# dschleef/schroedinger

Measured on AMD Instinct MI355X. Metric: Mpix/s IIWT+OBMC decode, 2160p s16, higher is better.
Workload: dtype s16

## Files before the change

### schroedinger_amd/csrc/frameops.hip

```cpp

#include "schro_hip_internal.h"
#include <type_traits>

namespace schro {
namespace {

constexpr int kThreads = 256;

__device__ __forceinline__ int
clampi (int x, int lo, int hi)
{
  return min (max (x, lo), hi);
}


constexpr int kCvtTW = 512, kCvtTH = 4;

template < typename T >
__device__ __forceinline__ uint8_t
offsetconvert (T s)
{
  if constexpr (sizeof (T) == 2) {
    int v = (int16_t) (s + 128);
    return (uint8_t) clampi (v, 0, 255);
  } else {
    int t = (int) ((unsigned) s + 128u);
    t = clampi (t, -32768, 32767);
    return (uint8_t) clampi (t, 0, 255);
  }
}

template < typename T >
__global__ __launch_bounds__ (kThreads)
void convert_kernel (const ConvertJob * __restrict__ jobs, int njobs)
{
  const int bid = xcd_tile_id (blockIdx.x, gridDim.x);
  const ConvertJob job = jobs[find_job (jobs, njobs, bid)];
  const int t = bid - job.tile_base;
  const int tx = t % job.tiles_x, ty = t / job.tiles_x;
  const int x = tx * kCvtTW + (threadIdx.x % 64) * 8;
  const int y = ty * kCvtTH + threadIdx.x / 64;
  if (y >= job.h || x >= job.w)
    return;
  const T *s = (const T *) ((const char *) job.src + (size_t) y * job.src_stride) + x;
  uint8_t *d = job.dst + (size_t) y * job.dst_stride + x;
  const bool vec = x + 8 <= job.w && (((uintptr_t) s & 15) == 0) && (((uintptr_t) d & 7) == 0);
  if (job.pred) {
    const uint8_t *p = job.pred + (size_t) y * job.pred_stride + x;
    for (int e = 0; e < 8 && x + e < job.w; e++)
      gstore < uint8_t > (d + e, combine_pred < T > (gload < T > (s + e), gload < uint8_t > (p + e)));
    return;
  }
  if (vec) {
    T v[8];
    if constexpr (sizeof (T) == 2) {
      *reinterpret_cast < u32x4 * >(v) = gload < u32x4 > (s);
    } else {
      reinterpret_cast < u32x4 * >(v)[0] = gload < u32x4 > (s);
      reinterpret_cast < u32x4 * >(v)[1] = gload < u32x4 > (s + 4);
    }
    uint32_t lo = 0, hi = 0;
#pragma unroll
    for (int e = 0; e < 4; e++) {
      lo |= (uint32_t) offsetconvert < T > (v[e]) << (8 * e);
      hi |= (uint32_t) offsetconvert < T > (v[4 + e]) << (8 * e);
    }
    gstore < u32x2 > (d, (u32x2) { lo, hi });
  } else {
    for (int e = 0; e < 8 && x + e < job.w; e++)
      gstore < uint8_t > (d + e, offsetconvert < T > (gload < T > (s + e)));
  }
}


constexpr int kUpTW = 128, kUpTH = 16;

typedef short short2v __attribute__ ((ext_vector_type (2)));

__device__ __forceinline__ short2v
lo_pair (uint32_t d)
{
  return __builtin_bit_cast (short2v, __builtin_amdgcn_perm (0u, d, 0x0c010c00u));
}

__device__ __forceinline__ short2v
hi_pair (uint32_t d)
{
  return __builtin_bit_cast (short2v, __builtin_amdgcn_perm (0u, d, 0x0c030c02u));
}

__device__ __forceinline__ short2v
mas8_pk (const short2v * r)
{
  short2v x = (r[3] + r[4]) * (short) 21 - (r[2] + r[5]) * (short) 7 + (r[1] + r[6]) * (short) 3
      - (r[0] + r[7]);
  x = (x + (short) 16) >> 5;
  x = __builtin_elementwise_max (x, (short2v) { 0, 0 });
  x = __builtin_elementwise_min (x, (short2v) { 255, 255 });
  return x;
}

__device__ __forceinline__ int
mas8_bytes (uint32_t lo4, uint32_t hi4)
{
  int acc = __builtin_amdgcn_sdot4 ((int) lo4, (int) 0x15f903ffu, 4096 + 16, false);
  acc = __builtin_amdgcn_sdot4 ((int) hi4, (int) 0xff03f915u, acc, false);
  return clampi (acc >> 5, 0, 255);
}

__device__ __forceinline__ void
mas8_row4 (uint32_t d0, uint32_t d1, uint32_t d2, int *out)
{
  out[0] = mas8_bytes (__builtin_amdgcn_alignbyte (d1, d0, 1), __builtin_amdgcn_alignbyte (d2, d1, 1));
  out[1] = mas8_bytes (__builtin_amdgcn_alignbyte (d1, d0, 2), __builtin_amdgcn_alignbyte (d2, d1, 2));
  out[2] = mas8_bytes (__builtin_amdgcn_alignbyte (d1, d0, 3), __builtin_amdgcn_alignbyte (d2, d1, 3));
  out[3] = mas8_bytes (d1, d2);
}

constexpr int kUpMaxLD = 2 * (kUpTW / 8 + 8);

template < bool PAIR > constexpr int kUpFetch = ((kUpTH + 7) * ((PAIR ? 2 : 1) * ((PAIR ? kUpTW / 2 : kUpTW) / 4 + 8) / 4) + kThreads - 1) / kThreads;

template < bool PAIR >
__device__ __forceinline__ void
upsample_fetch (const UpsampleJob & job, int t, u32x4 * q_out)
{
  constexpr int kTWp = PAIR ? kUpTW / 2 : kUpTW, kHalfLD = kTWp / 4 + 8;
  constexpr int kUpCh = (PAIR ? 2 : 1) * kHalfLD / 4, kHalfCh = kHalfLD / 4;
  const int tx = t % job.tiles_x, ty = t / job.tiles_x;
  const int x0 = tx * kTWp, y0 = ty * kUpTH;
  const int w = job.w, h = job.h;
  const int tid = threadIdx.x;
#pragma unroll
  for (int n = 0; n < kUpFetch < PAIR >; n++) {
    const int it = tid + n * kThreads;
    q_out[n] = (u32x4) { 0u, 0u, 0u, 0u };
    if (it >= (kUpTH + 7) * kUpCh)
      continue;
    const int ly = it / kUpCh, c = it - ly * kUpCh;
    const int half = PAIR ? c / kHalfCh : 0, cc = c - half * kHalfCh;
    const uint8_t *src = half ? job.src_b : job.src;
    const int sstride = half ? job.src_b_stride : job.src_stride;
    const bool src_al = ((((uintptr_t) src) | (uintptr_t) sstride) & 15) == 0;
    const int gy = clampi (y0 - 3 + ly, 0, h - 1);
    const int gx = x0 - 16 + 16 * cc;
    const uint8_t *row = src + (size_t) gy * sstride;
    u32x4 q;
    if (src_al && gx >= 0 && gx + 16 <= w) {
      q = gload < u32x4 > (row + gx);
    } else {
      uint32_t d[4] = { 0u, 0u, 0u, 0u };
#pragma unroll
      for (int k = 0; k < 16; k++)
        d[k >> 2] |= (uint32_t) gload < uint8_t > (row + clampi (gx + k, 0, w - 1)) << (8 * (k & 3));
      q = (u32x4) { d[0], d[1], d[2], d[3] };
    }
    q_out[n] = q;
  }
}

template < bool PAIR >
__device__ __forceinline__ void
upsample_stage (const u32x4 * q, uint32_t (*s0)[kUpMaxLD])
{
  constexpr int kTWp = PAIR ? kUpTW / 2 : kUpTW, kHalfLD = kTWp / 4 + 8, kUpCh = (PAIR ? 2 : 1) * kHalfLD / 4;
#pragma unroll
  for (int n = 0; n < kUpFetch < PAIR >; n++) {
    const int it = (int) threadIdx.x + n * kThreads;
    if (it < (kUpTH + 7) * kUpCh) {
      const int ly = it / kUpCh, c = it - ly * kUpCh;
      *reinterpret_cast < u32x4 * >(&s0[ly][4 * c]) = q[n];
    }
  }
}

template < bool PAIR >
__device__ __forceinline__ void
upsample_filter_store (const UpsampleJob & job, int t, uint32_t (*s0)[kUpMaxLD], uint32_t (*s2)[kUpMaxLD])
{
  constexpr int kTWp = PAIR ? kUpTW / 2 : kUpTW;
  constexpr int kHalfLD = kTWp / 4 + 8;
  constexpr int kHalfDW = kTWp / 4 + 2, kVDW = (PAIR ? 2 : 1) * kHalfDW;
  constexpr int ps = PAIR ? 1 : 0;
  static_assert ((PAIR ? 2 : 1) * kHalfLD <= kUpMaxLD, "LDS row");

  const int tx = t % job.tiles_x, ty = t / job.tiles_x;
  const int x0 = tx * kTWp, y0 = ty * kUpTH;
  const int w = job.w, h = job.h;
  const int tid = threadIdx.x;

  for (int it = tid; it < kUpTH * kVDW; it += kThreads) {
    const int gi = it % kVDW, ly = it / kVDW;
    const int half = PAIR ? gi / kHalfDW : 0, g = half * kHalfLD + (gi - half * kHalfDW) + 3;
    uint32_t out;
    if (y0 + ly >= h - 1) {
      out = s0[ly + 3][g];
    } else {
      short2v lo[8], hi[8];
#pragma unroll
      for (int k = 0; k < 8; k++) {
        const uint32_t d = s0[ly + k][g];
        lo[k] = lo_pair (d);
        hi[k] = hi_pair (d);
      }
      const short2v a = mas8_pk (lo), b = mas8_pk (hi);
      out = __builtin_amdgcn_perm (__builtin_bit_cast (uint32_t, b), __builtin_bit_cast (uint32_t, a), 0x06040200u);
    }
    s2[ly][g] = out;
  }
  __syncthreads ();

  static_assert ((kUpTW / 8) * kUpTH % kThreads == 0 && kUpTW / 8 == 16 && kUpTH % kHpBandRows == 0,
      "a lane per 8 pixels of 16 rows of the tile at a time");
  const int stride = job.dst_stride;
#pragma unroll 1
  for (int part = 0; part < (kUpTW / 8) * kUpTH / kThreads; part++) {
  const int ly = (tid >> 4) + part * (kThreads / 16), g8 = tid & 15;
  const int half = PAIR ? g8 >> 3 : 0, gg = PAIR ? g8 & 7 : g8;
  const int gx = x0 + 8 * gg, gy = y0 + ly;
  const int gd = half * kHalfLD + 2 * gg + 3;
  uint32_t pl[4][2];
  {
    const uint32_t a0 = s0[ly + 3][gd], a1 = s0[ly + 3][gd + 1], a2 = s0[ly + 3][gd + 2], a3 = s0[ly + 3][gd + 3];
    const uint32_t b0 = s2[ly][gd], b1 = s2[ly][gd + 1], b2 = s2[ly][gd + 2], b3 = s2[ly][gd + 3];
    constexpr uint32_t kS = 0x80808080u;
    int p1[8], p3[8];
    mas8_row4 (a0 ^ kS, a1 ^ kS, a2 ^ kS, p1);
    mas8_row4 (a1 ^ kS, a2 ^ kS, a3 ^ kS, p1 + 4);
    mas8_row4 (b0 ^ kS, b1 ^ kS, b2 ^ kS, p3);
    mas8_row4 (b1 ^ kS, b2 ^ kS, b3 ^ kS, p3 + 4);
    pl[0][0] = a1;
    pl[0][1] = a2;
    pl[2][0] = b1;
    pl[2][1] = b2;
    const bool edge_tile = x0 + kTWp >= w || y0 + kUpTH >= h;
#pragma unroll
    for (int hf = 0; hf < 2; hf++) {
      if (edge_tile) {
        pl[1][hf] = pl[3][hf] = 0;
#pragma unroll
        for (int e = 0; e < 4; e++) {
          const bool lastcol = gx + 4 * hf + e >= w - 1;
          int v1 = lastcol ? (int) ((pl[0][hf] >> (8 * e)) & 0xff) : p1[4 * hf + e];
          int v3 = lastcol ? (int) ((pl[2][hf] >> (8 * e)) & 0xff) : p3[4 * hf + e];
          if (gy >= h - 1)
            v3 = v1;
          pl[1][hf] |= (uint32_t) v1 << (8 * e);
          pl[3][hf] |= (uint32_t) v3 << (8 * e);
        }
      } else {
        pl[1][hf] = (uint32_t) p1[4 * hf] | ((uint32_t) p1[4 * hf + 1] << 8) | ((uint32_t) p1[4 * hf + 2] << 16)
            | ((uint32_t) p1[4 * hf + 3] << 24);
        pl[3][hf] = (uint32_t) p3[4 * hf] | ((uint32_t) p3[4 * hf + 1] << 8) | ((uint32_t) p3[4 * hf + 2] << 16)
            | ((uint32_t) p3[4 * hf + 3] << 24);
      }
    }
  }
  uint8_t *row = job.dst + hp_row_offset (min (gy, h - 1), stride);
  if constexpr (PAIR) {
    const int xb = 2 * (gx + kHpApron);
    const bool group_in = gx + 8 <= w;
#pragma unroll
    for (int p = 0; p < 4; p++) {
      const uint32_t n0 = (uint32_t) __builtin_amdgcn_mov_dpp ((int) pl[p][0], 0x128, 0xf, 0xf, true);
      const uint32_t n1 = (uint32_t) __builtin_amdgcn_mov_dpp ((int) pl[p][1], 0x128, 0xf, 0xf, true);
      if (group_in && gy < h) {
        const uint32_t u0 = half ? n0 : pl[p][0], u1 = half ? n1 : pl[p][1];
        const uint32_t v0 = half ? pl[p][0] : n0, v1 = half ? pl[p][1] : n1;
        const u32x4 v = (u32x4) { __builtin_amdgcn_perm (v0, u0, 0x05010400u), __builtin_amdgcn_perm (v0, u0, 0x07030602u),
          __builtin_amdgcn_perm (v1, u1, 0x05010400u), __builtin_amdgcn_perm (v1, u1, 0x07030602u) };
        gstore < u32x4 > (row + (size_t) ((xb >> 4) - half) * 512 + (size_t) (p * 128 + 16 * half), v);
      } else if (gy < h) {
        for (int e = 0; e < 8 && gx + e < w; e++) {
          const uint8_t v = (uint8_t) (pl[p][e >> 2] >> (8 * (e & 3)));
          const int xbe = xb + 2 * e + half;
          gstore < uint8_t > (row + hp_col_offset (xbe) + p * 128, v);
          gstore < uint8_t > (row + hp_col_offset (xbe - 16) + p * 128 + 16, v);
        }
      }
    }
  } else {
  const int odd = g8 & 1, xp16 = gx - 8 * odd + kHpApron;
  const bool pair_in = gx - 8 * odd + 16 <= w;
#pragma unroll
  for (int p = 0; p < 4; p++) {
    const uint32_t n0 = (uint32_t) __builtin_amdgcn_mov_dpp ((int) pl[p][0], 0xb1, 0xf, 0xf, true);
    const uint32_t n1 = (uint32_t) __builtin_amdgcn_mov_dpp ((int) pl[p][1], 0xb1, 0xf, 0xf, true);
    if (pair_in && gy < h) {
      const u32x4 v = odd ? (u32x4) { n0, n1, pl[p][0], pl[p][1] } : (u32x4) { pl[p][0], pl[p][1], n0, n1 };
      gstore < u32x4 > (row + (size_t) ((xp16 >> 4) - odd) * 512 + (size_t) (p * 128 + 16 * odd), v);
    } else if (gy < h) {
      for (int e = 0; e < 8 && gx + e < w; e++) {
        const uint8_t v = (uint8_t) (pl[p][e >> 2] >> (8 * (e & 3)));
        const int xp = gx + e + kHpApron;
        gstore < uint8_t > (row + hp_col_offset (xp) + p * 128, v);
        gstore < uint8_t > (row + hp_col_offset (xp - 16) + p * 128 + 16, v);
      }
    }
  }
  }
  }
  auto edge_dword = [&](int p, int r, int pos) {
    const uint32_t u = ((p < 2 ? s0[r + 3][pos >> 2] : s2[r][pos >> 2]) >> (8 * (pos & 3))) & 0xffu;
    if constexpr (!PAIR) {
      return u * 0x01010101u;
    } else {
      const uint32_t v = ((p < 2 ? s0[r + 3][kHalfLD + (pos >> 2)] : s2[r][kHalfLD + (pos >> 2)]) >> (8 * (pos & 3))) & 0xffu;
      return (u | (v << 8)) * 0x00010001u;
    }
  };
  if (x0 == 0) {
    constexpr int kPieces = 2 * ((kHpApron << ps) / 16) - 1;
    for (int it = tid; it < kUpTH * 4 * kPieces; it += kThreads) {
      const int piece = it % kPieces, p = (it / kPieces) & 3, r = it / (4 * kPieces);
      if (y0 + r >= h)
        continue;
      const uint32_t e = edge_dword (p, r, 16);
      uint8_t *d = job.dst + hp_row_offset (y0 + r, stride) + (size_t) ((piece >> 1) * 512 + 16 * (piece & 1)) + p * 128;
      gstore < u32x4 > (d, (u32x4) { e, e, e, e });
    }
  }
  if (x0 + kTWp >= w) {
    const int nch = stride >> 9, first = (w + kHpApron) << ps, c_lo = max (0, (first >> 4) - 1);
    const int ndw = (nch - c_lo) * 8;
    const int xl = w - 1 - (x0 - 16);
    for (int it = tid; it < kUpTH * 4 * ndw; it += kThreads) {
      const int dwi = it % ndw, p = (it / ndw) & 3, r = it / (4 * ndw);
      if (y0 + r >= h)
        continue;
      const int c = c_lo + (dwi >> 3), o = (dwi & 7) * 4, col = 16 * c + o;
      if (col + 3 < first)
        continue;
      const uint32_t e = edge_dword (p, r, xl);
      uint8_t *d = job.dst + hp_row_offset (y0 + r, stride) + (size_t) c * 512 + p * 128 + o;
      if (col >= first) {
        gstore < uint32_t > (d, e);
      } else {
        for (int k = first - col; k < 4; k++)
          gstore < uint8_t > (d + k, (uint8_t) (e >> (8 * k)));
      }
    }
  }
}

__global__ __launch_bounds__ (kThreads)
void upsample_kernel (const UpsampleJob * __restrict__ jobs, int njobs)
{
  __shared__ __attribute__ ((aligned (16))) uint32_t s0[kUpTH + 7][kUpMaxLD];
  __shared__ __attribute__ ((aligned (16))) uint32_t s2[kUpTH][kUpMaxLD];
  const int bid = xcd_tile_id (blockIdx.x, gridDim.x);
  const UpsampleJob job = jobs[find_job (jobs, njobs, bid)];
  if (job.src_b) {
    u32x4 q[kUpFetch < true >];
    upsample_fetch < true > (job, bid - job.tile_base, q);
    upsample_stage < true > (q, s0);
    __syncthreads ();
    upsample_filter_store < true > (job, bid - job.tile_base, s0, s2);
  } else {
    u32x4 q[kUpFetch < false >];
    upsample_fetch < false > (job, bid - job.tile_base, q);
    upsample_stage < false > (q, s0);
    __syncthreads ();
    upsample_filter_store < false > (job, bid - job.tile_base, s0, s2);
  }
}

#ifdef SCHRO_HIP_EXPERIMENTS
template < bool PAIR >
__device__ __forceinline__ void
upsample_persist_body (const UpsampleJob * __restrict__ jobs, int njobs, int total, uint32_t (*s0)[kUpMaxLD], uint32_t (*s2)[kUpMaxLD])
{
  u32x4 q[kUpFetch < PAIR >];
  int v = blockIdx.x;
  if (v >= total)
    return;
  int bid = xcd_tile_id (v, total);
  UpsampleJob job = jobs[find_job (jobs, njobs, bid)];
  upsample_fetch < PAIR > (job, bid - job.tile_base, q);
  for (;;) {
    upsample_stage < PAIR > (q, s0);
    __syncthreads ();
    const int vn = v + (int) gridDim.x;
    UpsampleJob jn = job;
    int bn = bid;
    if (vn < total) {
      bn = xcd_tile_id (vn, total);
      jn = jobs[find_job (jobs, njobs, bn)];
      upsample_fetch < PAIR > (jn, bn - jn.tile_base, q);
    }
    upsample_filter_store < PAIR > (job, bid - job.tile_base, s0, s2);
    if (vn >= total)
      break;
    __syncthreads ();
    v = vn;
    bid = bn;
    job = jn;
  }
}

__global__ __launch_bounds__ (kThreads)
void upsample_persist_kernel (const UpsampleJob * __restrict__ jobs, int njobs, int total)
{
  __shared__ __attribute__ ((aligned (16))) uint32_t s0[kUpTH + 7][kUpMaxLD];
  __shared__ __attribute__ ((aligned (16))) uint32_t s2[kUpTH][kUpMaxLD];
  if (jobs[0].src_b)
    upsample_persist_body < true > (jobs, njobs, total, s0, s2);
  else
    upsample_persist_body < false > (jobs, njobs, total, s0, s2);
}
#endif


constexpr int kPackGX = 64, kPackRows = 4;

__device__ __forceinline__ uint32_t
pack_sample (const PackJob & job, int comp, int t_hs, int X, int Y)
{
  int x, y;
  if (comp == 0) {
    x = min (X, job.sw - 1);
    y = min (Y, job.sh - 1);
  } else {
    const int sw = (job.sw + (1 << t_hs) - 1) >> t_hs;
    const int Xc = min (X, sw - 1), Yc = min (Y, job.sh - 1);
    x = t_hs == job.hs ? Xc : (t_hs > job.hs ? 2 * Xc : Xc >> 1);
    y = job.vs ? Yc >> 1 : Yc;
  }
  return gload < uint8_t > (job.src[comp] + (size_t) y * job.src_stride[comp] + x);
}

__device__ __forceinline__ uint32_t
v210_sample (const PackJob & job, int comp, int X, int Y)
{
  if (job.src_bpp == 1) {
    const uint32_t v = pack_sample (job, comp, 1, X, Y);
    return (v << 2) | (v >> 6);
  }
  const int cw = comp ? (job.sw + 1) >> 1 : job.sw;
  const int x = min (X, cw - 1), y = min (Y, job.sh - 1);
  const uint8_t *row = job.src[comp] + (size_t) y * job.src_stride[comp];
  const int v = job.src_bpp == 2 ? (int) gload < int16_t > ((const int16_t *) row + x)
      : (int) (int16_t) gload < int32_t > ((const int32_t *) row + x);
  return (uint32_t) clampi (v + 512, 0, 1023);
}

__device__ __forceinline__ int
wide_sample (const PackJob & job, int target_bpp, int t_hs, int comp, int X, int Y)
{
  const int cw = comp ? (job.sw + (1 << t_hs) - 1) >> t_hs : job.sw;
  const int x = min (X, cw - 1), y = min (Y, job.sh - 1);
  const uint8_t *row = job.src[comp] + (size_t) y * job.src_stride[comp];
  int v;
  if (job.src_bpp == 1)
    v = (int) gload < uint8_t > (row + x) - 128;
  else if (job.src_bpp == 2)
    v = gload < int16_t > ((const int16_t *) row + x);
  else
    v = gload < int32_t > ((const int32_t *) row + x);
  return target_bpp == 2 ? (int) (int16_t) v : v;
}

__device__ __forceinline__ uint32_t
v216_line_byte (const PackJob & job, int comp, int b, int Y)
{
  return ((uint32_t) (uint16_t) wide_sample (job, 2, 1, comp, b >> 1, Y) >> (8 * (b & 1))) & 0xffu;
}

__global__ __launch_bounds__ (kThreads)
void pack_kernel (const PackJob * __restrict__ jobs, int njobs)
{
  const int bid = xcd_tile_id (blockIdx.x, gridDim.x);
  const PackJob job = jobs[find_job (jobs, njobs, bid)];
  const int t = bid - job.tile_base;
  const int ty = fdiv (t, job.tiles_x), tx = t - ty * job.tiles_x;
  const int g = tx * kPackGX + (threadIdx.x & (kPackGX - 1));
  const int y = ty * kPackRows + (threadIdx.x >> 6);
  static_assert (kPackGX == 64 && kThreads == kPackGX * kPackRows, "one wave per packed row");
  if (y >= job.h)
    return;
  uint8_t *d = job.dst + (size_t) y * job.dst_stride + 16 * (size_t) g;
  uint32_t o[4];
  if (job.format == SCHRO_HIP_FORMAT_v210) {
    const int x0 = 6 * g;
    if (x0 >= job.w)
      return;
    uint32_t yv[6], cb[3], cr[3];
#pragma unroll
    for (int k = 0; k < 6; k++)
      yv[k] = x0 + k < job.w ? v210_sample (job, 0, x0 + k, y) : 0u;
#pragma unroll
    for (int k = 0; k < 3; k++) {
      const bool in = x0 + 2 * k < job.w;
      cb[k] = in ? v210_sample (job, 1, 3 * g + k, y) : 0u;
      cr[k] = in ? v210_sample (job, 2, 3 * g + k, y) : 0u;
    }
    o[0] = (cr[0] << 20) | (yv[0] << 10) | cb[0];
    o[1] = (yv[2] << 20) | (cb[1] << 10) | yv[1];
    o[2] = (cb[2] << 20) | (yv[3] << 10) | cr[1];
    o[3] = (yv[5] << 20) | (cr[2] << 10) | yv[4];
    if ((((uintptr_t) d) & 15) == 0) {
      gstore < u32x4 > (d, (u32x4) { o[0], o[1], o[2], o[3] });
    } else {
      for (int k = 0; k < 4; k++)
        gstore < u32_u > (d + 4 * k, o[k]);
    }
    return;
  }
  if (job.format == SCHRO_HIP_FORMAT_v216 || job.format == SCHRO_HIP_FORMAT_ARGB || job.format == SCHRO_HIP_FORMAT_AY64) {
    int nbytes = 16;
    if (job.format == SCHRO_HIP_FORMAT_v216) {
      const int pairs = job.w >> 1, j0 = 2 * g;
      if (j0 >= pairs)
        return;
#pragma unroll
      for (int k = 0; k < 2; k++) {
        const int j = j0 + k;
        const uint32_t u = v216_line_byte (job, 1, j, y), v = v216_line_byte (job, 2, j, y);
        const uint32_t y0 = v216_line_byte (job, 0, 2 * j, y), y1 = v216_line_byte (job, 0, 2 * j + 1, y);
        o[2 * k] = u * 0x0101u | (y0 * 0x0101u << 16);
        o[2 * k + 1] = v * 0x0101u | (y1 * 0x0101u << 16);
      }
      nbytes = 8 * min (2, pairs - j0);
    } else if (job.format == SCHRO_HIP_FORMAT_ARGB) {
      const int x0 = 4 * g;
      if (x0 >= job.w)
        return;
#pragma unroll
      for (int k = 0; k < 4; k++) {
        const int x = x0 + k;
        const int yv = wide_sample (job, 2, 0, 0, x, y), co = wide_sample (job, 2, 0, 1, x, y);
        const int cg = wide_sample (job, 2, 0, 2, x, y);
        const int t = yv + (cg >> 1), b = t - (co >> 1);
        o[k] = 0xffu | ((uint32_t) ((b + co) & 0xff) << 8) | ((uint32_t) ((t + cg) & 0xff) << 16)
            | ((uint32_t) (b & 0xff) << 24);
      }
      nbytes = 4 * min (4, job.w - x0);
    } else {
      const int x0 = 2 * g;
      if (x0 >= job.w)
        return;
#pragma unroll
      for (int k = 0; k < 2; k++) {
        const int x = x0 + k;
        uint32_t w[3];
#pragma unroll
        for (int c = 0; c < 3; c++) {
          const long long v = (long long) wide_sample (job, 4, 0, c, x, y) + 0x8000;
          w[c] = (uint32_t) (v < 0 ? 0 : (v > 0xffff ? 0xffff : v));
        }
        o[2 * k] = 0xffffu | (w[0] << 16);
        o[2 * k + 1] = w[1] | (w[2] << 16);
      }
      nbytes = 8 * min (2, job.w - x0);
    }
    if (nbytes == 16 && (((uintptr_t) d) & 15) == 0) {
      gstore < u32x4 > (d, (u32x4) { o[0], o[1], o[2], o[3] });
    } else {
      for (int b = 0; b < nbytes; b++)
        gstore < uint8_t > (d + b, (uint8_t) (o[b >> 2] >> (8 * (b & 3))));
    }
    return;
  }
  if (job.format == SCHRO_HIP_FORMAT_AYUV) {
    const int x0 = 4 * g;
    if (x0 >= job.w)
      return;
#pragma unroll
    for (int k = 0; k < 4; k++) {
      const int x = x0 + k;
      o[k] = 0xffu | (pack_sample (job, 0, 0, x, y) << 8) | (pack_sample (job, 1, 0, x, y) << 16)
          | (pack_sample (job, 2, 0, x, y) << 24);
    }
    const int n = min (4, job.w - x0);
    if (n == 4 && (((uintptr_t) d) & 15) == 0) {
      gstore < u32x4 > (d, (u32x4) { o[0], o[1], o[2], o[3] });
    } else {
      for (int k = 0; k < n; k++)
        for (int b = 0; b < 4; b++)
          gstore < uint8_t > (d + 4 * k + b, (uint8_t) (o[k] >> (8 * b)));
    }
  } else {
    const int p0 = 4 * g, pairs = job.w >> 1;
    if (p0 >= pairs)
      return;
    const bool yuyv = job.format == SCHRO_HIP_FORMAT_YUYV;
    const int cy = job.vs ? min (y, job.sh - 1) >> 1 : min (y, job.sh - 1);
    const uint8_t *py = job.src[0] + (size_t) min (y, job.sh - 1) * job.src_stride[0] + 2 * p0;
    const uint8_t *pu = job.src[1] + (size_t) cy * job.src_stride[1] + p0;
    const uint8_t *pv = job.src[2] + (size_t) cy * job.src_stride[2] + p0;
    if (job.hs == 1 && 2 * p0 + 8 <= job.sw && p0 + 4 <= pairs
        && ((((uintptr_t) py) & 7) | (((uintptr_t) pu) & 3) | (((uintptr_t) pv) & 3)) == 0) {
      const u32x2 yy = gload < u32x2 > (py);
      const uint32_t uu = gload < uint32_t > (pu), vv = gload < uint32_t > (pv);
      const uint32_t uv01 = __builtin_amdgcn_perm (vv, uu, 0x05010400u);
      const uint32_t uv23 = __builtin_amdgcn_perm (vv, uu, 0x07030602u);
      if (yuyv) {
        o[0] = __builtin_amdgcn_perm (uv01, yy.x, 0x05010400u);
        o[1] = __builtin_amdgcn_perm (uv01, yy.x, 0x07030602u);
        o[2] = __builtin_amdgcn_perm (uv23, yy.y, 0x05010400u);
        o[3] = __builtin_amdgcn_perm (uv23, yy.y, 0x07030602u);
      } else {
        o[0] = __builtin_amdgcn_perm (yy.x, uv01, 0x05010400u);
        o[1] = __builtin_amdgcn_perm (yy.x, uv01, 0x07030602u);
        o[2] = __builtin_amdgcn_perm (yy.y, uv23, 0x05010400u);
        o[3] = __builtin_amdgcn_perm (yy.y, uv23, 0x07030602u);
      }
      if ((((uintptr_t) d) & 15) == 0) {
        gstore < u32x4 > (d, (u32x4) { o[0], o[1], o[2], o[3] });
        return;
      }
    } else {
#pragma unroll
      for (int k = 0; k < 4; k++) {
        const int j = p0 + k;
        const uint32_t y0 = pack_sample (job, 0, 1, 2 * j, y), y1 = pack_sample (job, 0, 1, 2 * j + 1, y);
        const uint32_t u = pack_sample (job, 1, 1, j, y), v = pack_sample (job, 2, 1, j, y);
        o[k] = yuyv ? (y0 | (u << 8) | (y1 << 16) | (v << 24)) : (u | (y0 << 8) | (v << 16) | (y1 << 24));
      }
    }
    const int n = min (4, pairs - p0);
    for (int k = 0; k < n; k++)
      for (int b = 0; b < 4; b++)
        gstore < uint8_t > (d + 4 * k + b, (uint8_t) (o[k] >> (8 * b)));
  }
}

template < typename T >
__global__ __launch_bounds__ (kThreads)
void shift_right_kernel (const ConvertJob * __restrict__ jobs, int njobs, int shift)
{
  const int bid = blockIdx.x;
  const ConvertJob job = jobs[find_job (jobs, njobs, bid)];
  const int t = bid - job.tile_base;
  const int ty = fdiv (t, job.tiles_x), tx = t - ty * job.tiles_x;
  const int x = tx * kCvtTW + (threadIdx.x % 64) * 8;
  const int y = ty * kCvtTH + threadIdx.x / 64;
  if (y >= job.h || x >= job.w)
    return;
  typedef typename std::make_unsigned < T >::type U;
  const U rnd = (U) ((1u << shift) >> 1);
  T *row = (T *) ((char *) job.dst + (size_t) y * job.dst_stride);
  for (int e = 0; e < 8 && x + e < job.w; e++) {
    const T v = gload < T > (row + x + e);
    gstore < T > (row + x + e, (T) ((T) ((U) v + rnd) >> shift));
  }
}

template < typename S, bool SUB >
__global__ __launch_bounds__ (kThreads)
void add_kernel (const ConvertJob * __restrict__ jobs, int njobs)
{
  typedef short s16x2 __attribute__ ((ext_vector_type (2)));
  const int bid = blockIdx.x;
  const ConvertJob job = jobs[find_job (jobs, njobs, bid)];
  const int t = bid - job.tile_base;
  const int ty = fdiv (t, job.tiles_x), tx = t - ty * job.tiles_x;
  const int x = tx * kCvtTW + (threadIdx.x % 64) * 8;
  const int y = ty * kCvtTH + threadIdx.x / 64;
  if (y >= job.h || x >= job.w)
    return;
  int16_t *drow = (int16_t *) (job.dst + (size_t) y * job.dst_stride) + x;
  const S *srow = (const S *) ((const char *) job.src + (size_t) y * job.src_stride) + x;
  if (x + 8 <= job.w && (((uintptr_t) drow) & 15) == 0 && (((uintptr_t) srow) & (8 * sizeof (S) - 1)) == 0) {
    const u32x4 d = gload < u32x4 > (drow);
    uint32_t dv[4] = { d.x, d.y, d.z, d.w }, av[4];
    if constexpr (sizeof (S) == 2) {
      const u32x4 a = gload < u32x4 > (srow);
      av[0] = a.x;
      av[1] = a.y;
      av[2] = a.z;
      av[3] = a.w;
    } else {
      const u32x2 b = gload < u32x2 > (srow);
      av[0] = __builtin_amdgcn_perm (0u, b.x, 0x0c010c00u);
      av[1] = __builtin_amdgcn_perm (0u, b.x, 0x0c030c02u);
      av[2] = __builtin_amdgcn_perm (0u, b.y, 0x0c010c00u);
      av[3] = __builtin_amdgcn_perm (0u, b.y, 0x0c030c02u);
    }
#pragma unroll
    for (int k = 0; k < 4; k++) {
      const s16x2 a = __builtin_bit_cast (s16x2, dv[k]), b = __builtin_bit_cast (s16x2, av[k]);
      dv[k] = __builtin_bit_cast (uint32_t, (s16x2) (SUB ? a - b : a + b));
    }
    gstore < u32x4 > (drow, (u32x4) { dv[0], dv[1], dv[2], dv[3] });
    return;
  }
  for (int e = 0; e < 8 && x + e < job.w; e++) {
    const int16_t a = gload < int16_t > (drow + e), b = (int16_t) gload < S > (srow + e);
    gstore < int16_t > (drow + e, (int16_t) (SUB ? a - b : a + b));
  }
}

}

int
launch_shift_right (hipStream_t stream, const ConvertJob * d_jobs, int njobs, int total_tiles, int bpp, int shift)
{
  if (bpp == 2)
    SCHRO_LAUNCH ((shift_right_kernel < int16_t >), dim3 (total_tiles), dim3 (kThreads), 0, stream, d_jobs,
        njobs, shift);
  else
    SCHRO_LAUNCH ((shift_right_kernel < int32_t >), dim3 (total_tiles), dim3 (kThreads), 0, stream, d_jobs,
        njobs, shift);
  hipError_t e = hipGetLastError ();
  if (e != hipSuccess)
    return set_error (SCHRO_HIP_EDEVICE, "shift_right launch: %s", hipGetErrorString (e));
  return 0;
}

int
launch_add (hipStream_t stream, const ConvertJob * d_jobs, int njobs, int total_tiles, int src_bpp, bool subtract)
{
  if (src_bpp == 2 && subtract)
    SCHRO_LAUNCH ((add_kernel < int16_t, true >), dim3 (total_tiles), dim3 (kThreads), 0, stream, d_jobs, njobs);
  else if (subtract)
    SCHRO_LAUNCH ((add_kernel < uint8_t, true >), dim3 (total_tiles), dim3 (kThreads), 0, stream, d_jobs, njobs);
  else if (src_bpp == 2)
    SCHRO_LAUNCH ((add_kernel < int16_t, false >), dim3 (total_tiles), dim3 (kThreads), 0, stream, d_jobs, njobs);
  else
    SCHRO_LAUNCH ((add_kernel < uint8_t, false >), dim3 (total_tiles), dim3 (kThreads), 0, stream, d_jobs, njobs);
  hipError_t e = hipGetLastError ();
  if (e != hipSuccess)
    return set_error (SCHRO_HIP_EDEVICE, "add launch: %s", hipGetErrorString (e));
  return 0;
}

void
pack_tile_geometry (int *groups_x, int *rows)
{
  *groups_x = kPackGX;
  *rows = kPackRows;
}

int
launch_pack (hipStream_t stream, const PackJob * d_jobs, int njobs, int total_tiles)
{
  SCHRO_LAUNCH (pack_kernel, dim3 (total_tiles), dim3 (kThreads), 0, stream, d_jobs, njobs);
  hipError_t e = hipGetLastError ();
  if (e != hipSuccess)
    return set_error (SCHRO_HIP_EDEVICE, "pack launch: %s", hipGetErrorString (e));
  return 0;
}

void
convert_tile_geometry (int *tw, int *th)
{
  *tw = kCvtTW;
  *th = kCvtTH;
}

int
launch_convert (hipStream_t stream, const ConvertJob * d_jobs, int njobs, int total_tiles, int bpp)
{
  if (bpp == 2)
    SCHRO_LAUNCH ((convert_kernel < int16_t >), dim3 (total_tiles), dim3 (kThreads), 0,
        stream, d_jobs, njobs);
  else
    SCHRO_LAUNCH ((convert_kernel < int32_t >), dim3 (total_tiles), dim3 (kThreads), 0,
        stream, d_jobs, njobs);
  hipError_t e = hipGetLastError ();
  if (e != hipSuccess)
    return set_error (SCHRO_HIP_EDEVICE, "convert launch: %s", hipGetErrorString (e));
  return 0;
}

void
upsample_tile_geometry (int *tw, int *th)
{
  *tw = kUpTW;
  *th = kUpTH;
}

int
launch_upsample (hipStream_t stream, const UpsampleJob * d_jobs, int njobs, int total_tiles, int persist_grid)
{
#ifdef SCHRO_HIP_EXPERIMENTS
  if (persist_grid > 0 && persist_grid < total_tiles)
    SCHRO_LAUNCH (upsample_persist_kernel, dim3 (persist_grid), dim3 (kThreads), 0, stream, d_jobs, njobs, total_tiles);
  else
#endif
  SCHRO_LAUNCH (upsample_kernel, dim3 (total_tiles), dim3 (kThreads), 0, stream, d_jobs,
      njobs);
  hipError_t e = hipGetLastError ();
  if (e != hipSuccess)
    return set_error (SCHRO_HIP_EDEVICE, "upsample launch: %s", hipGetErrorString (e));
  return 0;
}

}
```

Baseline: 196,800.

## Restructure upsample filter: row-grouped vertical pass, early plane stores, packed clamps

The vertical half-pel pass now has each lane compute four output rows from eleven LDS reads, so loaded taps are reused across neighbouring rows instead of being reloaded eight times per row. The store phase drops its per-part loop and writes integer-position planes 0 and 2 before the horizontal filters run, so the global stores can overlap the arithmetic. Horizontal results are saturated with packed convert and v_sat_pk_u8_i16 instead of scalar clamps. Experiment-only env variants (stores-only and filters-only) and per-step template switches were added for profiling. One risk is that only part of the lanes are busy in the vertical pass.

```diff
diff --git a/schroedinger_amd/csrc/frameops.hip b/schroedinger_amd/csrc/frameops.hip
--- a/schroedinger_amd/csrc/frameops.hip
+++ b/schroedinger_amd/csrc/frameops.hip
@@ -1,5 +1,6 @@
 
 #include "schro_hip_internal.h"
+#include <cstring>
 #include <type_traits>
 
 namespace schro {
@@ -104,8 +105,7 @@
 mas8_bytes (uint32_t lo4, uint32_t hi4)
 {
   int acc = __builtin_amdgcn_sdot4 ((int) lo4, (int) 0x15f903ffu, 4096 + 16, false);
-  acc = __builtin_amdgcn_sdot4 ((int) hi4, (int) 0xff03f915u, acc, false);
-  return clampi (acc >> 5, 0, 255);
+  return __builtin_amdgcn_sdot4 ((int) hi4, (int) 0xff03f915u, acc, false);
 }
 
 __device__ __forceinline__ void
@@ -115,6 +115,28 @@
   out[1] = mas8_bytes (__builtin_amdgcn_alignbyte (d1, d0, 2), __builtin_amdgcn_alignbyte (d2, d1, 2));
   out[2] = mas8_bytes (__builtin_amdgcn_alignbyte (d1, d0, 3), __builtin_amdgcn_alignbyte (d2, d1, 3));
   out[3] = mas8_bytes (d1, d2);
+}
+
+__device__ __forceinline__ int
+mas8_sample (int sum)
+{
+  return clampi (sum >> 5, 0, 255);
+}
+
+__device__ __forceinline__ uint32_t
+sat_pair_u8 (short2v x)
+{
+  uint32_t r;
+  asm ("v_sat_pk_u8_i16 %0, %1":"=v" (r):"v" (__builtin_bit_cast (uint32_t, x)));
+  return r;
+}
+
+__device__ __forceinline__ uint32_t
+mas8_samples4 (const int *sum)
+{
+  const short2v lo = __builtin_amdgcn_cvt_pk_i16 (sum[0], sum[1]) >> (short2v) { 5, 5 };
+  const short2v hi = __builtin_amdgcn_cvt_pk_i16 (sum[2], sum[3]) >> (short2v) { 5, 5 };
+  return __builtin_amdgcn_perm (sat_pair_u8 (hi), sat_pair_u8 (lo), 0x05040100u);
 }
 
 constexpr int kUpMaxLD = 2 * (kUpTW / 8 + 8);
@@ -174,7 +196,12 @@
   }
 }
 
-template < bool PAIR >
+enum { kUpFull = 0, kUpStoresOnly = 1, kUpFiltersOnly = 2 };
+
+enum { kUpEarlyStores = 1, kUpRowGroups = 2, kUpPackedClamp = 4 };
+constexpr int kUpSteps = kUpEarlyStores | kUpRowGroups | kUpPackedClamp;
+
+template < bool PAIR, int MODE, int STEPS >
 __device__ __forceinline__ void
 upsample_filter_store (const UpsampleJob & job, int t, uint32_t (*s0)[kUpMaxLD], uint32_t (*s2)[kUpMaxLD])
 {
@@ -189,116 +216,147 @@
   const int w = job.w, h = job.h;
   const int tid = threadIdx.x;
 
-  for (int it = tid; it < kUpTH * kVDW; it += kThreads) {
-    const int gi = it % kVDW, ly = it / kVDW;
-    const int half = PAIR ? gi / kHalfDW : 0, g = half * kHalfLD + (gi - half * kHalfDW) + 3;
-    uint32_t out;
-    if (y0 + ly >= h - 1) {
-      out = s0[ly + 3][g];
-    } else {
-      short2v lo[8], hi[8];
-#pragma unroll
-      for (int k = 0; k < 8; k++) {
-        const uint32_t d = s0[ly + k][g];
-        lo[k] = lo_pair (d);
-        hi[k] = hi_pair (d);
-      }
-      const short2v a = mas8_pk (lo), b = mas8_pk (hi);
-      out = __builtin_amdgcn_perm (__builtin_bit_cast (uint32_t, b), __builtin_bit_cast (uint32_t, a), 0x06040200u);
-    }
-    s2[ly][g] = out;
+  static_assert ((kUpTW / 8) * kUpTH == kThreads && kUpTW / 8 == 16 && kUpTH % kHpBandRows == 0,
+      "a lane per 8 pixels of one row of the tile");
+  const int stride = job.dst_stride;
+  const int ly = tid >> 4, g8 = tid & 15;
+  const int shalf = PAIR ? g8 >> 3 : 0, gg = PAIR ? g8 & 7 : g8;
+  const int gx = x0 + 8 * gg, gy = y0 + ly;
+  const int gd = shalf * kHalfLD + 2 * gg + 3;
+  uint8_t *row = job.dst + hp_row_offset (min (gy, h - 1), stride);
+  uint32_t kept[4] = { 0u, 0u, 0u, 0u };
+  auto store_plane = [&](int p, uint32_t d0, uint32_t d1) {
+    if constexpr (MODE == kUpFiltersOnly) {
+      kept[p] = d0 ^ d1;
+    } else if constexpr (PAIR) {
+      const int xb = 2 * (gx + kHpApron);
+      const bool group_in = gx + 8 <= w;
+      const uint32_t n0 = (uint32_t) __builtin_amdgcn_mov_dpp ((int) d0, 0x128, 0xf, 0xf, true);
+      const uint32_t n1 = (uint32_t) __builtin_amdgcn_mov_dpp ((int) d1, 0x128, 0xf, 0xf, true);
+      if (group_in && gy < h) {
+        const uint32_t u0 = shalf ? n0 : d0, u1 = shalf ? n1 : d1;
+        const uint32_t v0 = shalf ? d0 : n0, v1 = shalf ? d1 : n1;
+        const u32x4 v = (u32x4) { __builtin_amdgcn_perm (v0, u0, 0x05010400u), __builtin_amdgcn_perm (v0, u0, 0x07030602u),
+          __builtin_amdgcn_perm (v1, u1, 0x05010400u), __builtin_amdgcn_perm (v1, u1, 0x07030602u) };
+        gstore < u32x4 > (row + (size_t) ((xb >> 4) - shalf) * 512 + (size_t) (p * 128 + 16 * shalf), v);
+      } else if (gy < h) {
+        for (int e = 0; e < 8 && gx + e < w; e++) {
+          const uint8_t v = (uint8_t) ((e < 4 ? d0 : d1) >> (8 * (e & 3)));
+          const int xbe = xb + 2 * e + shalf;
+          gstore < uint8_t > (row + hp_col_offset (xbe) + p * 128, v);
+          gstore < uint8_t > (row + hp_col_offset (xbe - 16) + p * 128 + 16, v);
+        }
+      }
+    } else {
+      const int odd = g8 & 1, xp16 = gx - 8 * odd + kHpApron;
+      const bool pair_in = gx - 8 * odd + 16 <= w;
+      const uint32_t n0 = (uint32_t) __builtin_amdgcn_mov_dpp ((int) d0, 0xb1, 0xf, 0xf, true);
+      const uint32_t n1 = (uint32_t) __builtin_amdgcn_mov_dpp ((int) d1, 0xb1, 0xf, 0xf, true);
+      if (pair_in && gy < h) {
+        const u32x4 v = odd ? (u32x4) { n0, n1, d0, d1 } : (u32x4) { d0, d1, n0, n1 };
+        gstore < u32x4 > (row + (size_t) ((xp16 >> 4) - odd) * 512 + (size_t) (p * 128 + 16 * odd), v);
+      } else if (gy < h) {
+        for (int e = 0; e < 8 && gx + e < w; e++) {
+          const uint8_t v = (uint8_t) ((e < 4 ? d0 : d1) >> (8 * (e & 3)));
+          const int xp = gx + e + kHpApron;
+          gstore < uint8_t > (row + hp_col_offset (xp) + p * 128, v);
+          gstore < uint8_t > (row + hp_col_offset (xp - 16) + p * 128 + 16, v);
+        }
+      }
+    }
+  };
+
+  if constexpr ((STEPS & kUpEarlyStores) != 0)
+    store_plane (0, s0[ly + 3][gd + 1], s0[ly + 3][gd + 2]);
+
+  if constexpr ((STEPS & kUpRowGroups) != 0 && MODE != kUpStoresOnly) {
+    static_assert (kUpTH == 16 && 4 * kVDW <= kThreads, "four groups of 4 rows");
+    if (tid < 4 * kVDW) {
+      const int gi = tid % kVDW, r0 = 4 * (tid / kVDW);
+      const int half = PAIR ? gi / kHalfDW : 0, g = half * kHalfLD + (gi - half * kHalfDW) + 3;
+      uint32_t d[11];
+      short2v ev[11], od[11];
+#pragma unroll
+      for (int k = 0; k < 11; k++) {
+        d[k] = s0[r0 + k][g];
+        ev[k] = __builtin_bit_cast (short2v, d[k] & 0x00ff00ffu);
+        od[k] = __builtin_bit_cast (short2v, (d[k] >> 8) & 0x00ff00ffu);
+      }
+#pragma unroll
+      for (int j = 0; j < 4; j++) {
+        const uint32_t a = __builtin_bit_cast (uint32_t, mas8_pk (ev + j)), b = __builtin_bit_cast (uint32_t, mas8_pk (od + j));
+        s2[r0 + j][g] = y0 + r0 + j >= h - 1 ? d[j + 3] : (a | (b << 8));
+      }
+    }
+  } else {
+    for (int it = tid; it < kUpTH * kVDW; it += kThreads) {
+      const int gi = it % kVDW, vy = it / kVDW;
+      const int half = PAIR ? gi / kHalfDW : 0, g = half * kHalfLD + (gi - half * kHalfDW) + 3;
+      uint32_t out;
+      if (MODE == kUpStoresOnly || y0 + vy >= h - 1) {
+        out = s0[vy + 3][g];
+      } else {
+        short2v lo[8], hi[8];
+#pragma unroll
+        for (int k = 0; k < 8; k++) {
+          const uint32_t d = s0[vy + k][g];
+          lo[k] = lo_pair (d);
+          hi[k] = hi_pair (d);
+        }
+        const short2v a = mas8_pk (lo), b = mas8_pk (hi);
+        out = __builtin_amdgcn_perm (__builtin_bit_cast (uint32_t, b), __builtin_bit_cast (uint32_t, a), 0x06040200u);
+      }
+      s2[vy][g] = out;
+    }
   }
   __syncthreads ();
 
-  static_assert ((kUpTW / 8) * kUpTH % kThreads == 0 && kUpTW / 8 == 16 && kUpTH % kHpBandRows == 0,
-      "a lane per 8 pixels of 16 rows of the tile at a time");
-  const int stride = job.dst_stride;
-#pragma unroll 1
-  for (int part = 0; part < (kUpTW / 8) * kUpTH / kThreads; part++) {
-  const int ly = (tid >> 4) + part * (kThreads / 16), g8 = tid & 15;
-  const int half = PAIR ? g8 >> 3 : 0, gg = PAIR ? g8 & 7 : g8;
-  const int gx = x0 + 8 * gg, gy = y0 + ly;
-  const int gd = half * kHalfLD + 2 * gg + 3;
-  uint32_t pl[4][2];
   {
     const uint32_t a0 = s0[ly + 3][gd], a1 = s0[ly + 3][gd + 1], a2 = s0[ly + 3][gd + 2], a3 = s0[ly + 3][gd + 3];
     const uint32_t b0 = s2[ly][gd], b1 = s2[ly][gd + 1], b2 = s2[ly][gd + 2], b3 = s2[ly][gd + 3];
-    constexpr uint32_t kS = 0x80808080u;
-    int p1[8], p3[8];
-    mas8_row4 (a0 ^ kS, a1 ^ kS, a2 ^ kS, p1);
-    mas8_row4 (a1 ^ kS, a2 ^ kS, a3 ^ kS, p1 + 4);
-    mas8_row4 (b0 ^ kS, b1 ^ kS, b2 ^ kS, p3);
-    mas8_row4 (b1 ^ kS, b2 ^ kS, b3 ^ kS, p3 + 4);
-    pl[0][0] = a1;
-    pl[0][1] = a2;
-    pl[2][0] = b1;
-    pl[2][1] = b2;
-    const bool edge_tile = x0 + kTWp >= w || y0 + kUpTH >= h;
-#pragma unroll
-    for (int hf = 0; hf < 2; hf++) {
-      if (edge_tile) {
-        pl[1][hf] = pl[3][hf] = 0;
-#pragma unroll
-        for (int e = 0; e < 4; e++) {
-          const bool lastcol = gx + 4 * hf + e >= w - 1;
-          int v1 = lastcol ? (int) ((pl[0][hf] >> (8 * e)) & 0xff) : p1[4 * hf + e];
-          int v3 = lastcol ? (int) ((pl[2][hf] >> (8 * e)) & 0xff) : p3[4 * hf + e];
-          if (gy >= h - 1)
-            v3 = v1;
-          pl[1][hf] |= (uint32_t) v1 << (8 * e);
-          pl[3][hf] |= (uint32_t) v3 << (8 * e);
+    if constexpr ((STEPS & kUpEarlyStores) != 0)
+      store_plane (2, b1, b2);
+    uint32_t h1[2] = { a1, a2 }, h3[2] = { b1, b2 };
+    if constexpr (MODE != kUpStoresOnly) {
+      constexpr uint32_t kS = 0x80808080u;
+      int p1[8], p3[8];
+      mas8_row4 (a0 ^ kS, a1 ^ kS, a2 ^ kS, p1);
+      mas8_row4 (a1 ^ kS, a2 ^ kS, a3 ^ kS, p1 + 4);
+      mas8_row4 (b0 ^ kS, b1 ^ kS, b2 ^ kS, p3);
+      mas8_row4 (b1 ^ kS, b2 ^ kS, b3 ^ kS, p3 + 4);
+      const bool edge_tile = x0 + kTWp >= w || y0 + kUpTH >= h;
+#pragma unroll
+      for (int hf = 0; hf < 2; hf++) {
+        const uint32_t i0 = h1[hf], i2 = h3[hf];
+        if (edge_tile) {
+          h1[hf] = h3[hf] = 0;
+#pragma unroll
+          for (int e = 0; e < 4; e++) {
+            const bool lastcol = gx + 4 * hf + e >= w - 1;
+            int v1 = lastcol ? (int) ((i0 >> (8 * e)) & 0xff) : mas8_sample (p1[4 * hf + e]);
+            int v3 = lastcol ? (int) ((i2 >> (8 * e)) & 0xff) : mas8_sample (p3[4 * hf + e]);
+            if (gy >= h - 1)
+              v3 = v1;
+            h1[hf] |= (uint32_t) v1 << (8 * e);
+            h3[hf] |= (uint32_t) v3 << (8 * e);
+          }
+        } else {
+          h1[hf] = mas8_samples4 (p1 + 4 * hf);
+          h3[hf] = mas8_samples4 (p3 + 4 * hf);
         }
-      } else {
-        pl[1][hf] = (uint32_t) p1[4 * hf] | ((uint32_t) p1[4 * hf + 1] << 8) | ((uint32_t) p1[4 * hf + 2] << 16)
-            | ((uint32_t) p1[4 * hf + 3] << 24);
-        pl[3][hf] = (uint32_t) p3[4 * hf] | ((uint32_t) p3[4 * hf + 1] << 8) | ((uint32_t) p3[4 * hf + 2] << 16)
-            | ((uint32_t) p3[4 * hf + 3] << 24);
-      }
-    }
-  }
-  uint8_t *row = job.dst + hp_row_offset (min (gy, h - 1), stride);
-  if constexpr (PAIR) {
-    const int xb = 2 * (gx + kHpApron);
-    const bool group_in = gx + 8 <= w;
-#pragma unroll
-    for (int p = 0; p < 4; p++) {
-      const uint32_t n0 = (uint32_t) __builtin_amdgcn_mov_dpp ((int) pl[p][0], 0x128, 0xf, 0xf, true);
-      const uint32_t n1 = (uint32_t) __builtin_amdgcn_mov_dpp ((int) pl[p][1], 0x128, 0xf, 0xf, true);
-      if (group_in && gy < h) {
-        const uint32_t u0 = half ? n0 : pl[p][0], u1 = half ? n1 : pl[p][1];
-        const uint32_t v0 = half ? pl[p][0] : n0, v1 = half ? pl[p][1] : n1;
-        const u32x4 v = (u32x4) { __builtin_amdgcn_perm (v0, u0, 0x05010400u), __builtin_amdgcn_perm (v0, u0, 0x07030602u),
-          __builtin_amdgcn_perm (v1, u1, 0x05010400u), __builtin_amdgcn_perm (v1, u1, 0x07030602u) };
-        gstore < u32x4 > (row + (size_t) ((xb >> 4) - half) * 512 + (size_t) (p * 128 + 16 * half), v);
-      } else if (gy < h) {
-        for (int e = 0; e < 8 && gx + e < w; e++) {
-          const uint8_t v = (uint8_t) (pl[p][e >> 2] >> (8 * (e & 3)));
-          const int xbe = xb + 2 * e + half;
-          gstore < uint8_t > (row + hp_col_offset (xbe) + p * 128, v);
-          gstore < uint8_t > (row + hp_col_offset (xbe - 16) + p * 128 + 16, v);
-        }
-      }
-    }
-  } else {
-  const int odd = g8 & 1, xp16 = gx - 8 * odd + kHpApron;
-  const bool pair_in = gx - 8 * odd + 16 <= w;
-#pragma unroll
-  for (int p = 0; p < 4; p++) {
-    const uint32_t n0 = (uint32_t) __builtin_amdgcn_mov_dpp ((int) pl[p][0], 0xb1, 0xf, 0xf, true);
-    const uint32_t n1 = (uint32_t) __builtin_amdgcn_mov_dpp ((int) pl[p][1], 0xb1, 0xf, 0xf, true);
-    if (pair_in && gy < h) {
-      const u32x4 v = odd ? (u32x4) { n0, n1, pl[p][0], pl[p][1] } : (u32x4) { pl[p][0], pl[p][1], n0, n1 };
-      gstore < u32x4 > (row + (size_t) ((xp16 >> 4) - odd) * 512 + (size_t) (p * 128 + 16 * odd), v);
-    } else if (gy < h) {
-      for (int e = 0; e < 8 && gx + e < w; e++) {
-        const uint8_t v = (uint8_t) (pl[p][e >> 2] >> (8 * (e & 3)));
-        const int xp = gx + e + kHpApron;
-        gstore < uint8_t > (row + hp_col_offset (xp) + p * 128, v);
-        gstore < uint8_t > (row + hp_col_offset (xp - 16) + p * 128 + 16, v);
-      }
-    }
-  }
-  }
+      }
+    }
+    if constexpr ((STEPS & kUpEarlyStores) == 0)
+      store_plane (0, a1, a2);
+    store_plane (1, h1[0], h1[1]);
+    if constexpr ((STEPS & kUpEarlyStores) == 0)
+      store_plane (2, b1, b2);
+    store_plane (3, h3[0], h3[1]);
+  }
+  if constexpr (MODE == kUpFiltersOnly) {
+    if (gy < h && gx + 8 <= w)
+      gstore < u32x4 > (row + hp_col_offset (((gx & ~15) + kHpApron) << ps) + (size_t) (16 * (g8 & 1)), (u32x4) { kept[0], kept[1], kept[2], kept[3] });
+    return;
   }
   auto edge_dword = [&](int p, int r, int pos) {
     const uint32_t u = ((p < 2 ? s0[r + 3][pos >> 2] : s2[r][pos >> 2]) >> (8 * (pos & 3))) & 0xffu;
@@ -343,6 +401,7 @@
   }
 }
 
+template < int MODE, int STEPS >
 __global__ __launch_bounds__ (kThreads)
 void upsample_kernel (const UpsampleJob * __restrict__ jobs, int njobs)
 {
@@ -355,13 +414,13 @@
     upsample_fetch < true > (job, bid - job.tile_base, q);
     upsample_stage < true > (q, s0);
     __syncthreads ();
-    upsample_filter_store < true > (job, bid - job.tile_base, s0, s2);
+    upsample_filter_store < true, MODE, STEPS > (job, bid - job.tile_base, s0, s2);
   } else {
     u32x4 q[kUpFetch < false >];
     upsample_fetch < false > (job, bid - job.tile_base, q);
     upsample_stage < false > (q, s0);
     __syncthreads ();
-    upsample_filter_store < false > (job, bid - job.tile_base, s0, s2);
+    upsample_filter_store < false, MODE, STEPS > (job, bid - job.tile_base, s0, s2);
   }
 }
 
@@ -388,7 +447,7 @@
       jn = jobs[find_job (jobs, njobs, bn)];
       upsample_fetch < PAIR > (jn, bn - jn.tile_base, q);
     }
-    upsample_filter_store < PAIR > (job, bid - job.tile_base, s0, s2);
+    upsample_filter_store < PAIR, kUpFull, kUpSteps > (job, bid - job.tile_base, s0, s2);
     if (vn >= total)
       break;
     __syncthreads ();
@@ -775,12 +834,27 @@
 launch_upsample (hipStream_t stream, const UpsampleJob * d_jobs, int njobs, int total_tiles, int persist_grid)
 {
 #ifdef SCHRO_HIP_EXPERIMENTS
+  static const char *const vname = SCHRO_ENV ("SCHRO_HIP_UPSAMPLE_VARIANT"), *const sname = SCHRO_ENV ("SCHRO_HIP_UPSAMPLE_STEPS");
+  static const int variant = !vname ? kUpFull : !strcmp (vname, "stores") ? kUpStoresOnly : !strcmp (vname, "filters") ? kUpFiltersOnly : kUpFull;
+  static const int steps = sname ? atoi (sname) : kUpSteps;
+  const dim3 grid (total_tiles), block (kThreads);
   if (persist_grid > 0 && persist_grid < total_tiles)
-    SCHRO_LAUNCH (upsample_persist_kernel, dim3 (persist_grid), dim3 (kThreads), 0, stream, d_jobs, njobs, total_tiles);
+    SCHRO_LAUNCH (upsample_persist_kernel, dim3 (persist_grid), block, 0, stream, d_jobs, njobs, total_tiles);
+  else if (variant == kUpStoresOnly)
+    SCHRO_LAUNCH ((upsample_kernel < kUpStoresOnly, kUpSteps >), grid, block, 0, stream, d_jobs, njobs);
+  else if (variant == kUpFiltersOnly)
+    SCHRO_LAUNCH ((upsample_kernel < kUpFiltersOnly, kUpSteps >), grid, block, 0, stream, d_jobs, njobs);
+  else if (steps == (kUpEarlyStores | kUpRowGroups | kUpPackedClamp))
+    SCHRO_LAUNCH ((upsample_kernel < kUpFull, kUpEarlyStores | kUpRowGroups | kUpPackedClamp >), grid, block, 0, stream, d_jobs, njobs);
+  else if (steps == kUpEarlyStores)
+    SCHRO_LAUNCH ((upsample_kernel < kUpFull, kUpEarlyStores >), grid, block, 0, stream, d_jobs, njobs);
+  else if (steps == kUpRowGroups)
+    SCHRO_LAUNCH ((upsample_kernel < kUpFull, kUpRowGroups >), grid, block, 0, stream, d_jobs, njobs);
+  else if (steps == kUpPackedClamp)
+    SCHRO_LAUNCH ((upsample_kernel < kUpFull, kUpPackedClamp >), grid, block, 0, stream, d_jobs, njobs);
   else
 #endif
-  SCHRO_LAUNCH (upsample_kernel, dim3 (total_tiles), dim3 (kThreads), 0, stream, d_jobs,
-      njobs);
+  SCHRO_LAUNCH ((upsample_kernel < kUpFull, kUpSteps >), dim3 (total_tiles), dim3 (kThreads), 0, stream, d_jobs, njobs);
   hipError_t e = hipGetLastError ();
   if (e != hipSuccess)
     return set_error (SCHRO_HIP_EDEVICE, "upsample launch: %s", hipGetErrorString (e));
```

After: 199,400 (median of 6 runs). Within noise of the previous version (+1.3%).
